# avlmaps/AVLMaps

Hardware: AMD Instinct MI355X
Metric: voxel_query_similarities_per_sec (higher is better)
Workload: dtype f32

## Files before the change

avlmaps_amd/csrc/avl_builder.hip:

```cpp
#include <algorithm>
#include <climits>
#include <cstring>
#include <vector>

#include "avl_builder_state.h"

namespace avl {

#ifdef AVL_PROBE_CHAIN
__device__ unsigned long long* g_probe = nullptr;
constexpr int kProbeK12Row0 = 16384;
#define AVL_STAMP(var)                                                                                             \
    unsigned long long var;                                                                                        \
    asm volatile("s_waitcnt vmcnt(0) lgkmcnt(0)\n\ts_memrealtime %0\n\ts_waitcnt lgkmcnt(0)" : "=s"(var)::"memory")
#define AVL_STAMP_DECL(var) unsigned long long var = 0
#define AVL_RESTAMP(var) asm volatile("s_waitcnt vmcnt(0) lgkmcnt(0)\n\ts_memrealtime %0\n\ts_waitcnt lgkmcnt(0)" : "=s"(var)::"memory")
#else
#define AVL_STAMP(var)
#define AVL_STAMP_DECL(var)
#define AVL_RESTAMP(var)
#endif

#ifndef AVL_K3_THREADS
#define AVL_K3_THREADS 256
#endif
constexpr int kFuseWaves = 128;

constexpr int kEmpty = -1, kPending = -2;
constexpr int kAggregateSamples = 32768;
constexpr int kMaxPendingSpins = 1 << 18;

template <int LINES>
__device__ __forceinline__ void warm_kernel_arguments() {
#ifndef AVL_NO_KERNARG_WARMUP
    static_assert(LINES == 4 || LINES == 8 || LINES == 12 || LINES == 16, "four lines per step");
    const auto p = __builtin_amdgcn_kernarg_segment_ptr();
    int t0, t1, t2, t3;
    if constexpr (LINES == 4)
        asm volatile("s_load_dword %0, %4, 0x0\n s_load_dword %1, %4, 0x40\n s_load_dword %2, %4, 0x80\n s_load_dword %3, %4, 0xc0\n"
                     "s_waitcnt lgkmcnt(0)" : "=&s"(t0), "=&s"(t1), "=&s"(t2), "=&s"(t3) : "s"(p));
    if constexpr (LINES == 8)
        asm volatile("s_load_dword %0, %4, 0x0\n s_load_dword %1, %4, 0x40\n s_load_dword %2, %4, 0x80\n s_load_dword %3, %4, 0xc0\n"
                     "s_load_dword %0, %4, 0x100\n s_load_dword %1, %4, 0x140\n s_load_dword %2, %4, 0x180\n s_load_dword %3, %4, 0x1c0\n"
                     "s_waitcnt lgkmcnt(0)" : "=&s"(t0), "=&s"(t1), "=&s"(t2), "=&s"(t3) : "s"(p));
    if constexpr (LINES == 12)
        asm volatile("s_load_dword %0, %4, 0x0\n s_load_dword %1, %4, 0x40\n s_load_dword %2, %4, 0x80\n s_load_dword %3, %4, 0xc0\n"
                     "s_load_dword %0, %4, 0x100\n s_load_dword %1, %4, 0x140\n s_load_dword %2, %4, 0x180\n s_load_dword %3, %4, 0x1c0\n"
                     "s_load_dword %0, %4, 0x200\n s_load_dword %1, %4, 0x240\n s_load_dword %2, %4, 0x280\n s_load_dword %3, %4, 0x2c0\n"
                     "s_waitcnt lgkmcnt(0)" : "=&s"(t0), "=&s"(t1), "=&s"(t2), "=&s"(t3) : "s"(p));
    if constexpr (LINES == 16)
        asm volatile("s_load_dword %0, %4, 0x0\n s_load_dword %1, %4, 0x40\n s_load_dword %2, %4, 0x80\n s_load_dword %3, %4, 0xc0\n"
                     "s_load_dword %0, %4, 0x100\n s_load_dword %1, %4, 0x140\n s_load_dword %2, %4, 0x180\n s_load_dword %3, %4, 0x1c0\n"
                     "s_load_dword %0, %4, 0x200\n s_load_dword %1, %4, 0x240\n s_load_dword %2, %4, 0x280\n s_load_dword %3, %4, 0x2c0\n"
                     "s_load_dword %0, %4, 0x300\n s_load_dword %1, %4, 0x340\n s_load_dword %2, %4, 0x380\n s_load_dword %3, %4, 0x3c0\n"
                     "s_waitcnt lgkmcnt(0)" : "=&s"(t0), "=&s"(t1), "=&s"(t2), "=&s"(t3) : "s"(p));
    (void)t0; (void)t1; (void)t2; (void)t3;
    __builtin_amdgcn_sched_barrier(0);
#endif
}

__device__ __forceinline__ int py_int(double v) {
    return (int)fmin(fmax(v, -2.0e9), 2.0e9);
}

__device__ __forceinline__ double gemv3(const double* a, double x0, double x1, double x2) {
    return fma(a[2], x2, fma(a[0], x0, a[1] * x1));
}

struct SampleRec {
    double alpha;
    int32_t cell, fpix;
    uint32_t rgbv;
    int32_t slot;
};

template <int THREADS, int MODE = 0>
__device__ __forceinline__ SampleRec bp_voxelize_body(int blk, const FrameParams& fp, const float* depth,
                                                      const int32_t* __restrict__ sample_idx, const uint8_t* rgb,
                                                      int32_t* __restrict__ cell_slot, int32_t* __restrict__ slot_cell, const Recs& recs,
                                                      unsigned long long* __restrict__ counters, int* __restrict__ err_flags,
                                                      PreRec* __restrict__ pre_out = nullptr) {
    __shared__ unsigned blk_new;
    __shared__ unsigned long long blk_base;
    if constexpr (MODE != 2) {
        if (threadIdx.x == 0) blk_new = 0;
        __syncthreads();
    }
    const int s = blk * THREADS + threadIdx.x;
    const bool valid = s < fp.P;
    AVL_STAMP(pt0);
    AVL_STAMP_DECL(pt1);
    AVL_STAMP_DECL(pt2);
    AVL_STAMP_DECL(pt3);
    double alpha = 0.0;
    int32_t cell = -1, fpix = 0;
    uint32_t rgbv = 0;
    int32_t seen = kEmpty;
    bool ok = false, err_box = false, err_img = false;
    uint8_t c0 = 0, c1 = 0, c2 = 0;
    if constexpr (MODE == 1) {
        const PreRec r = valid ? fp.pre[s] : PreRec{0.0, -1, 0, 0u, 0u};
        alpha = r.alpha;
        cell = r.cell;
        fpix = r.fpix;
        rgbv = r.rgbv;
        ok = cell >= 0;
        err_box = (r.flags & 1u) != 0;
        err_img = (r.flags & 2u) != 0;
        AVL_RESTAMP(pt1);
        seen = cell_slot[ok ? cell : 0];
        AVL_RESTAMP(pt2);
        AVL_RESTAMP(pt3);
    } else {

    const BatchEntry* be = fp.batch ? fp.batch + (valid ? s / fp.P_frame : 0) : nullptr;
    double T[12];
    if (be) {
#pragma unroll
        for (int k = 0; k < 12; ++k) T[k] = be->t[k];
        depth = be->depth;
        rgb = be->rgb;
    } else {
#pragma unroll
        for (int k = 0; k < 12; ++k) T[k] = fp.t[k];
    }
    const int pix = !valid ? -1 : (be ? be->samples[s % fp.P_frame] : sample_idx[s]);
    const bool ok0 = pix >= 0 && pix < fp.H * fp.W;
    AVL_RESTAMP(pt1);
    const int pixc = ok0 ? pix : 0;
    const float* dsrc = ok0 ? depth : reinterpret_cast<const float*>(cell_slot);
    const double x = (double)(pixc % fp.W) + 0.5, y = (double)(pixc / fp.W) + 0.5;
    const double z = fp.depth_u16 ? (double)reinterpret_cast<const uint16_t*>(dsrc)[pixc] / fp.depth_div : (double)dsrc[pixc];
    const double pl0 = fma(fp.kinv[2], 1.0, fma(fp.kinv[1], y, fp.kinv[0] * x)) * z;
    const double pl1 = fma(fp.kinv[5], 1.0, fma(fp.kinv[4], y, fp.kinv[3] * x)) * z;
    const double pl2 = fma(fp.kinv[8], 1.0, fma(fp.kinv[7], y, fp.kinv[6] * x)) * z;
    const bool ok1 = ok0 && (pl2 > fp.min_depth) && (pl2 < fp.max_depth);
    AVL_RESTAMP(pt2);
    const double g0 = fma(T[3], 1.0, fma(T[2], pl2, fma(T[1], pl1, T[0] * pl0)));
    const double g1 = fma(T[7], 1.0, fma(T[6], pl2, fma(T[5], pl1, T[4] * pl0)));
    const double g2 = fma(T[11], 1.0, fma(T[10], pl2, fma(T[9], pl1, T[8] * pl0)));
    int row, col, h;
    if (fp.mode == 0) {
        row = py_int(fp.half_gs - (double)py_int(g0 / fp.cs));
        col = py_int(fp.half_gs - (double)py_int(g1 / fp.cs));
        h = py_int(g2 / fp.cs);
    } else {
        row = py_int(rint((g0 - fp.pcd_min[0]) / fp.cs));
        h = py_int(rint((g1 - fp.pcd_min[1]) / fp.cs));
        col = py_int(rint((g2 - fp.pcd_min[2]) / fp.cs));
    }
    const bool in_grid = !(col >= fp.n1 || row >= fp.n0 || h >= fp.n2 || col < 0 || row < 0 || h < 0);
    const bool ok2 = ok1 && in_grid;
    err_box = ok1 && !in_grid && fp.mode == 1;
    const int32_t cell_try = ok2 ? (int32_t)(((unsigned)row * (unsigned)fp.n1 + (unsigned)col) * (unsigned)fp.n2 + (unsigned)h) : 0;
    if constexpr (MODE == 0) seen = cell_slot[cell_try];
    __builtin_amdgcn_sched_barrier(0);
    double q0 = gemv3(fp.k + 0, pl0, pl1, pl2), q1 = gemv3(fp.k + 3, pl0, pl1, pl2), q2 = gemv3(fp.k + 6, pl0, pl1, pl2);
    int px = py_int(q0 / q2 - 0.5), py = py_int(q1 / q2 - 0.5);
    px += px < 0 ? fp.W : 0;
    py += py < 0 ? fp.H : 0;
    const bool in_img = !(px < 0 || px >= fp.W || py < 0 || py >= fp.H);
    err_img = ok2 && !in_img;
    const bool ok3 = ok2 && in_img;
    const size_t rgb_off = ok3 ? ((size_t)py * fp.W + px) * 3 : 0;
    using gbyte_ptr = const __attribute__((address_space(1))) uint8_t*;
    const gbyte_ptr c = (gbyte_ptr)(ok3 ? rgb + rgb_off : reinterpret_cast<const uint8_t*>(cell_slot));
    c0 = c[0];
    c1 = c[1];
    c2 = c[2];
    __builtin_amdgcn_sched_barrier(0);
    q0 = gemv3(fp.kf + 0, pl0, pl1, pl2);
    q1 = gemv3(fp.kf + 3, pl0, pl1, pl2);
    q2 = gemv3(fp.kf + 6, pl0, pl1, pl2);
    px = py_int(q0 / q2 - 0.5);
    py = py_int(q1 / q2 - 0.5);
    ok = ok3 && !(px < 0 || py < 0 || px >= fp.Wf || py >= fp.Hf);
    if (ok2) fpix = (int32_t)((unsigned)py * (unsigned)fp.Wf + (unsigned)px);
    const double radial = (pl0 * pl0 + pl1 * pl1) + pl2 * pl2;
    const double alpha_try = exp(-radial / fp.two_sigma_sq);
    if (ok) {
        alpha = alpha_try;
        cell = cell_try;
    }
// ... 7 lines not shown
    }
    int32_t known = -1;
    bool creator = false;
    if (ok) {
        if (seen == kEmpty) creator = atomicCAS(&cell_slot[cell], kEmpty, kPending) == kEmpty;
        else if (seen >= 0) known = seen;
    }
    AVL_STAMP(pt4);
    const unsigned long long cmask = __ballot(creator);
    const int lane = threadIdx.x & 63;
    unsigned long long base = 0;
#ifndef AVL_K1_AGG_MIN
#define AVL_K1_AGG_MIN kAggregateSamples
#endif
    if (fp.P >= AVL_K1_AGG_MIN) {
        unsigned woff = 0;
        if (cmask) {
            const int leader = __ffsll((long long)cmask) - 1;
            if (lane == leader) woff = atomicAdd(&blk_new, (unsigned)__popcll(cmask));
            woff = __shfl(woff, leader, 64);
        }
        __syncthreads();
        if (threadIdx.x == 0 && blk_new) blk_base = atomicAdd(&counters[0], (unsigned long long)blk_new);
        __syncthreads();
        base = blk_base + woff;
    } else if (cmask) {
        const int leader = __ffsll((long long)cmask) - 1;
        if (lane == leader) base = atomicAdd(&counters[0], (unsigned long long)__popcll(cmask));
        base = __shfl(base, leader, 64);
    }
    if (creator) {
        const unsigned long long slot = base + __popcll(cmask & ((1ull << lane) - 1ull));
        if ((long long)slot >= fp.capacity) {
            atomicOr(err_flags, 1);
            __hip_atomic_store(&cell_slot[cell], kEmpty, __ATOMIC_RELAXED, __HIP_MEMORY_SCOPE_AGENT);
        } else {
            slot_cell[slot] = cell;
            __hip_atomic_store(&cell_slot[cell], (int32_t)slot, __ATOMIC_RELAXED, __HIP_MEMORY_SCOPE_AGENT);
            known = (int32_t)slot;
        }
    }
    if (MODE == 0 && ok) rgbv = (uint32_t)c0 | ((uint32_t)c1 << 8) | ((uint32_t)c2 << 16);
    if (valid) {
        recs.alpha[s] = alpha;
        recs.fpix[s] = fpix;
        recs.rgb[s] = rgbv;
    }
    if (err_box) atomicOr(err_flags, 8);
    if (err_img) atomicOr(err_flags, 2);
#ifdef AVL_PROBE_CHAIN
    {
        AVL_STAMP(pt5);
        if (g_probe && valid && fp.P < kProbeK12Row0) {
            unsigned long long* q = g_probe + (size_t)(kProbeK12Row0 + s) * 8;
            q[0] = pt0; q[1] = pt1; q[2] = pt2; q[3] = pt3; q[4] = pt4; q[5] = pt5;
        }
    }
#endif
    return SampleRec{alpha, cell, fpix, rgbv, known};
}

template <bool MAY_COMPACT = true, int THREADS = 256>
__device__ __forceinline__ void link_body(int blk, int P, const int32_t* __restrict__ cell_slot, int32_t* __restrict__ head,
                                          const Recs& recs, unsigned long long* __restrict__ counters, const ReplayLog& log,
                                          long long log_base, unsigned long long frame_key, const BatchEntry* __restrict__ batch,
                                          int P_frame, const SampleRec& in, int* __restrict__ err_flags, const OwnerList& ol = OwnerList{}) {
    __shared__ unsigned blk_cnt[2];
    __shared__ unsigned sh_own[4];
    if (threadIdx.x < 2) blk_cnt[threadIdx.x] = 0;
    __syncthreads();
    const int s = blk * THREADS + threadIdx.x;
    const bool valid = s < P;
    int32_t slot = -1, next = -1;
    uint8_t owner = 0;
    if (valid) {
        const int32_t cell = in.cell;
        if (cell >= 0) {
            {
                slot = in.slot >= 0 ? in.slot : __hip_atomic_load(&cell_slot[cell], __ATOMIC_RELAXED, __HIP_MEMORY_SCOPE_AGENT);
                for (int spins = 0; slot == kPending; ++spins) {
                    if (spins >= kMaxPendingSpins) {
                        atomicOr(err_flags, 16);
                        slot = -1;
                        break;
                    }
                    __builtin_amdgcn_s_sleep(2);
                    slot = __hip_atomic_load(&cell_slot[cell], __ATOMIC_RELAXED, __HIP_MEMORY_SCOPE_AGENT);
                }
            }
            if (slot >= 0) {
                next = atomicExch(&head[slot], s);
                owner = next == -1;
            }
        }
    }
    const unsigned long long amask = __ballot(slot >= 0);
    const unsigned long long omask = __ballot(owner != 0);
    if (amask && (threadIdx.x & 63) == __ffsll((long long)amask) - 1) {
        atomicAdd(&blk_cnt[0], (unsigned)__popcll(amask));
        if (omask) atomicAdd(&blk_cnt[1], (unsigned)__popcll(omask));
    }
    if (MAY_COMPACT && (threadIdx.x & 63) == 0) sh_own[threadIdx.x >> 6] = (unsigned)__popcll(omask);
    if (valid) {
        recs.slot[s] = slot;
        recs.next[s] = next;
        recs.owner[s] = owner;
        if (log.slot) {
            const long long i = log_base + s;
            log.slot[i] = slot >= 0 ? (uint32_t)slot : 0xFFFFFFFFu;
#ifdef AVL_ABL_NOLOGREC
            if (false) {
#elif defined(AVL_LOG_UNCOND)
            {
#else
            if (slot >= 0) {
#endif
                const unsigned long long k = batch ? (batch[s / P_frame].frame_key | (unsigned)(s % P_frame)) : (frame_key | (unsigned)s);
                using u64x2 = __attribute__((ext_vector_type(2))) unsigned long long;
                u64x2* r = reinterpret_cast<u64x2*>(log.rec + i);
                r[0] = u64x2{(unsigned long long)__double_as_longlong(in.alpha), k};
                r[1] = u64x2{(unsigned long long)in.rgbv, 0ull};
            }
        }
    }
#ifdef AVL_PROBE_CHAIN
    {
        AVL_STAMP(pt7);
        if (g_probe && valid && P < kProbeK12Row0) g_probe[(size_t)(kProbeK12Row0 + s) * 8 + 7] = pt7 | ((unsigned long long)(slot >= 0) << 63);
    }
#endif
    __syncthreads();
    if (MAY_COMPACT && owner && P >= kAggregateSamples) {
        unsigned pos = (unsigned)__popcll(omask & ((1ull << (threadIdx.x & 63)) - 1ull));
        for (int w = 0; w < (int)(threadIdx.x >> 6); ++w) pos += sh_own[w];
        const size_t o = (size_t)blk * 256 + pos;
        ol.o_s[o] = s;
        ol.o_slot[o] = slot;
        ol.o_alpha[o] = in.alpha;
        ol.o_fpix[o] = in.fpix;
        ol.o_rgb[o] = in.rgbv;
    }
    if (MAY_COMPACT && P >= kAggregateSamples && threadIdx.x == 0) ol.ocnt[blk] = (int32_t)(sh_own[0] + sh_own[1] + sh_own[2] + sh_own[3]);
    if (threadIdx.x < 2 && blk_cnt[threadIdx.x]) atomicAdd(&counters[1 + threadIdx.x], (unsigned long long)blk_cnt[threadIdx.x]);
}

__global__ __launch_bounds__(256) void voxelize_link_kernel(FrameParams fp, const float* depth, const int32_t* __restrict__ sample_idx,
                                                            const uint8_t* rgb, int32_t* __restrict__ cell_slot,
                                                            int32_t* __restrict__ slot_cell, Recs recs, int32_t* __restrict__ head,
                                                            unsigned long long* __restrict__ counters, int* __restrict__ err_flags,
                                                            ReplayLog log, long long log_base, unsigned long long frame_key, OwnerList ol) {
    warm_kernel_arguments<12>();
    const SampleRec r = bp_voxelize_body<256>(blockIdx.x, fp, depth, sample_idx, rgb, cell_slot, slot_cell, recs, counters, err_flags);
    link_body<true, 256>(blockIdx.x, fp.P, cell_slot, head, recs, counters, log, log_base, frame_key, fp.batch, fp.P_frame, r, err_flags, ol);
}

__global__ __launch_bounds__(256) void voxelize_link_next_kernel(FrameParams fp, const float* depth, const int32_t* __restrict__ sample_idx,
                                                                 const uint8_t* rgb, int32_t* __restrict__ cell_slot,
                                                                 int32_t* __restrict__ slot_cell, Recs recs, int32_t* __restrict__ head,
                                                                 unsigned long long* __restrict__ counters, int* __restrict__ err_flags,
                                                                 ReplayLog log, long long log_base, unsigned long long frame_key,
                                                                 FrameParams fpn, PreGather next, int gb) {
    if ((int)blockIdx.x < gb) {
        bp_voxelize_body<256, 2>((int)blockIdx.x, fpn, next.depth, next.samples, next.rgb, cell_slot, slot_cell, recs, counters, err_flags, next.out);
        return;
    }
    const int blk = (int)blockIdx.x - gb;
    warm_kernel_arguments<12>();
    SampleRec r;
    if (fp.pre) r = bp_voxelize_body<256, 1>(blk, fp, depth, sample_idx, rgb, cell_slot, slot_cell, recs, counters, err_flags);
    else r = bp_voxelize_body<256, 0>(blk, fp, depth, sample_idx, rgb, cell_slot, slot_cell, recs, counters, err_flags);
    link_body<false, 256>(blk, fp.P, cell_slot, head, recs, counters, log, log_base, frame_key, nullptr, fp.P_frame, r, err_flags);
}

template <int CH, bool FULL>
__device__ __forceinline__ void fuse_group_impl(int s0, int32_t slot, double alpha0, int32_t fpix0, uint32_t rgb0, int P, int D_rt, unsigned long long frame_key, const BatchEntry* __restrict__ batch,
                                                int P_frame, const Recs& recs, int32_t* __restrict__ head, const float* __restrict__ feat,
                                                double* __restrict__ sum_feat, double* __restrict__ sum_w4,
                                                float* __restrict__ first_feat, double* __restrict__ first_alpha,
                                                unsigned long long* __restrict__ slot_key, uint8_t* __restrict__ dirty) {
    const int D = FULL ? 256 * CH : D_rt;
    const int lane = threadIdx.x & 63;
    AVL_STAMP(pt0);
    AVL_STAMP(pt1);
    const bool is_new = slot_key[slot] == kNoKey;
    const int h0 = head[slot];
    double* sf = sum_feat + (size_t)slot * D;
    AVL_STAMP(pt2);
#ifdef AVL_PROBE_CHAIN
    int probe_n = 1;
    unsigned long long pt3 = 0, pt4 = 0;
#endif

    double acc[CH][4], old[CH][4];
    float f1[CH][4];
#pragma unroll
    for (int c = 0; c < CH; ++c)
#pragma unroll
        for (int e = 0; e < 4; ++e) { acc[c][e] = 0.0; f1[c][e] = 0.f; old[c][e] = 0.0; }
    double w4 = 0.0, a1 = 0.0, w4_old = 0.0;
    int min_s = INT_MAX;
    if (!is_new) {
#pragma unroll
        for (int c = 0; c < CH; ++c) {
            const int d = c * 256 + lane * 4;
            if (FULL || (d + 3 < D && (D & 1) == 0)) {
                const double2 q0 = *reinterpret_cast<const double2*>(sf + d), q1 = *reinterpret_cast<const double2*>(sf + d + 2);
                old[c][0] = q0.x; old[c][1] = q0.y; old[c][2] = q1.x; old[c][3] = q1.y;
            } else {
#pragma unroll
                for (int e = 0; e < 4; ++e)
                    if (d + e < D) old[c][e] = sf[d + e];
            }
        }
    }
    if (lane < 4) w4_old = is_new ? 0.0 : sum_w4[(size_t)slot * 4 + lane];

    auto row_of = [&](int cur, int32_t fpix) { return (batch ? batch[cur / P_frame].feat : feat) + (size_t)fpix * D; };
    auto load_row = [&](float (&v)[CH][4], const float* f) {
#pragma unroll
        for (int c = 0; c < CH; ++c) {
            const int d = c * 256 + lane * 4;
            if (FULL || (d + 3 < D && (D & 3) == 0)) {
                const float4 q = *reinterpret_cast<const float4*>(f + d);
                v[c][0] = q.x; v[c][1] = q.y; v[c][2] = q.z; v[c][3] = q.w;
            } else {
#pragma unroll
                for (int e = 0; e < 4; ++e) v[c][e] = d + e < D ? f[d + e] : 0.f;
            }
        }
    };
    auto add = [&](int cur, double alpha, uint32_t rgbv, const float (&v)[CH][4]) {
        const bool first = cur < min_s;
        const bool hold = first && is_new;
        const bool rejoin = hold && min_s != INT_MAX;
        const double a_prev = a1;
        if (first) { min_s = cur; a1 = alpha; }
#pragma unroll
        for (int c = 0; c < CH; ++c) {
            if (FULL || c * 256 + lane * 4 < D) {
#pragma unroll
                for (int e = 0; e < 4; ++e) {
                    if (rejoin) acc[c][e] += a_prev * (double)f1[c][e];
                    if (!hold) acc[c][e] += alpha * (double)v[c][e];
                    if (first) f1[c][e] = v[c][e];
                }
            }
        }
        if (lane < 4) w4 += lane == 0 ? alpha : alpha * (double)((rgbv >> (8 * (lane - 1))) & 0xffu);
    };
    const float* feat0 = row_of(s0, fpix0);
#ifdef AVL_ABL_K3_SINGLE
    if (true) {
#else
    if (h0 == s0) {
#endif
        float v[CH][4];
        load_row(v, feat0);
        add(s0, alpha0, rgb0, v);
#ifdef AVL_PROBE_CHAIN
        { AVL_STAMP(ptx); pt3 = pt4 = ptx; }
#endif
    } else {
        int my = lane == 0 ? s0 : INT_MAX;
        int n = 1, cur = h0;
        while (cur != s0 && n < 64 && (unsigned)cur < (unsigned)P) {
            if (lane == n) my = cur;
            ++n;
            cur = recs.next[cur];
        }
#ifdef AVL_PROBE_CHAIN
        { AVL_STAMP(ptx); pt3 = ptx; probe_n = n; }
#endif
        double a_l = 0.0;
        int32_t fp_l = 0;
        uint32_t rgb_l = 0;
        if (lane < n) {
            a_l = recs.alpha[my];
            fp_l = recs.fpix[my];
            rgb_l = recs.rgb[my];
        }
#ifdef AVL_PROBE_CHAIN
        { AVL_STAMP(ptx); pt4 = ptx; }
#endif
        int rank = 0;
        for (int j = 0; j < n; ++j) rank += __builtin_amdgcn_readlane(my, j) < my ? 1 : 0;
        const int a_lo = __double2loint(a_l), a_hi = __double2hiint(a_l);
#ifndef AVL_K3_MR
#define AVL_K3_MR 2
#endif
        constexpr int MR = CH <= 4 ? AVL_K3_MR : 1;
        for (int k0 = 0; k0 < n; k0 += MR) {
            float v[MR][CH][4];
            int cj[MR], lj[MR];
#pragma unroll
            for (int j = 0; j < MR; ++j) {
                const unsigned long long m = __ballot(lane < n && rank == k0 + j);
                lj[j] = m ? __builtin_amdgcn_readfirstlane(__ffsll((long long)m) - 1) : 0;
                cj[j] = m ? __builtin_amdgcn_readlane(my, lj[j]) : -1;
                load_row(v[j], cj[j] >= 0 ? row_of(cj[j], __builtin_amdgcn_readlane(fp_l, lj[j])) : feat0);
            }
#pragma unroll
            for (int j = 0; j < MR; ++j) {
                if (cj[j] >= 0) {
                    const double al = __hiloint2double(__builtin_amdgcn_readlane(a_hi, lj[j]), __builtin_amdgcn_readlane(a_lo, lj[j]));
                    add(cj[j], al, (uint32_t)__builtin_amdgcn_readlane((int)rgb_l, lj[j]), v[j]);
                }
            }
        }
        for (int steps = 0; cur != s0 && (unsigned)cur < (unsigned)P && steps < P; ++steps) {
            const int nxt = recs.next[cur];
            float v[CH][4];
            load_row(v, row_of(cur, recs.fpix[cur]));
            add(cur, recs.alpha[cur], recs.rgb[cur], v);
            cur = nxt;
        }
    }

    AVL_STAMP(pt5);
    float* ff = first_feat + (size_t)slot * D;
#pragma unroll
    for (int c = 0; c < CH; ++c) {
        const int d = c * 256 + lane * 4;
        double r[4];
#pragma unroll
// ... 395 lines not shown
    const unsigned gb = next.out ? (unsigned)((fpn.P + AVL_K3_THREADS - 1) / AVL_K3_THREADS) : 0u;
    hipLaunchKernelGGL(pipe_kernel<CH>, dim3(pb + wb + gb), dim3(AVL_K3_THREADS), 0, st, fp, (int)pb, reinterpret_cast<const float*>(d_depth), d_sample_idx,
                       d_rgb, b->cell_slot, b->slot_cell, b->recs, b->head, b->counters, b->err_flags, b->log, b->log_used, frame_key, prev,
                       b->D, b->sum_feat, b->sum_w4, b->first_feat, b->first_alpha, b->slot_key, b->dirty, fpn, next, (int)gb);
}

extern "C" {

#ifdef AVL_PROBE_CHAIN
__attribute__((visibility("default"))) int avl_debug_set_probe(void* d_buf) {
    AVL_HIP_CHECK(hipDeviceSynchronize());
    unsigned long long* p = reinterpret_cast<unsigned long long*>(d_buf);
    AVL_HIP_CHECK(hipMemcpyToSymbol(HIP_SYMBOL(avl::g_probe), &p, sizeof(p)));
    return AVL_OK;
}
#endif

int avl_builder_reset(avl_builder* b, void* stream) {
    AVL_REQUIRE(b, "avl_builder_reset: null handle");
    hipStream_t st = as_stream(stream);
    AVL_HIP_CHECK(hipMemsetAsync(b->cell_slot, 0xFF, b->ncell * sizeof(int32_t), st));
    AVL_HIP_CHECK(hipMemsetAsync(b->head, 0xFF, (size_t)b->capacity * sizeof(int32_t), st));
    AVL_HIP_CHECK(hipMemsetAsync(b->head_alt, 0xFF, (size_t)b->capacity * sizeof(int32_t), st));
    b->pend = avl_builder::Pending{};
    b->pre_held.valid = false;
    AVL_HIP_CHECK(hipMemsetAsync(b->dirty, 0, (size_t)b->capacity, st));
    AVL_HIP_CHECK(hipMemsetAsync(b->slot_cell, 0xFF, (size_t)b->capacity * sizeof(int32_t), st));
    AVL_HIP_CHECK(hipMemsetAsync(b->slot_key, 0xFF, (size_t)b->capacity * sizeof(unsigned long long), st));
    AVL_HIP_CHECK(hipMemsetAsync(b->counters, 0, 4 * sizeof(unsigned long long), st));
    AVL_HIP_CHECK(hipMemsetAsync(b->err_flags, 0, sizeof(int), st));
    b->key_bias = 0;
    b->log_used = 0;
    b->vox_bound = 0;
    drop_log_segments(b, st);
    return AVL_OK;
}

int avl_builder_destroy(avl_builder* b) {
    if (!b) return AVL_OK;
    drop_log_segments(b, nullptr);
    (void)hipFree(b->cell_slot); (void)hipFree(b->slot_cell); (void)hipFree(b->slot_key); (void)hipFree(b->sum_feat);
    (void)hipFree(b->sum_w4); (void)hipFree(b->first_feat); (void)hipFree(b->first_alpha); (void)hipFree(b->head);
    (void)hipFree(b->head_alt);
    (void)hipFree(b->dirty);
    (void)hipFree(b->counters); (void)hipFree(b->err_flags); (void)hipFree(b->recs_mem);
    (void)hipFree(b->log.slot); (void)hipFree(b->log.rec);
    (void)hipFree(b->rs_mem);
    (void)hipFree(b->d_table);
    delete b;
    return AVL_OK;
}

int avl_builder_create_grid(avl_builder** h_out, int n0, int gs, int vh, double cs, int D, int64_t capacity) {
    AVL_REQUIRE(h_out, "avl_builder_create: null output");
    *h_out = nullptr;
    avl::keep_mempool_once();
    avl_merge2_load();
    AVL_REQUIRE(n0 > 0 && gs > 0 && vh > 0 && D > 0 && cs > 0 && capacity > 0, "avl_builder_create: bad parameters");
    const double ncell_d = (double)n0 * gs * vh;
    AVL_REQUIRE(ncell_d < 2.0e9, "avl_builder_create: gs*gs*vh = %.0f cells exceeds the int32 cell index", ncell_d);
    AVL_REQUIRE(capacity < (1ll << 31), "avl_builder_create: capacity must fit int32 voxel ids");
    avl_builder* b = new avl_builder();
    b->n0 = n0; b->gs = gs; b->vh = vh; b->D = D; b->cs = cs; b->capacity = capacity;
    b->ncell = (size_t)n0 * gs * vh;
    hipError_t e = hipSuccess;
    auto alloc = [&](void** p, size_t bytes) { if (e == hipSuccess) e = hipMalloc(p, bytes); };
    alloc((void**)&b->cell_slot, b->ncell * sizeof(int32_t));
    alloc((void**)&b->slot_cell, (size_t)capacity * sizeof(int32_t));
    alloc((void**)&b->slot_key, (size_t)capacity * sizeof(unsigned long long));
    alloc((void**)&b->sum_feat, (size_t)capacity * D * sizeof(double));
    alloc((void**)&b->sum_w4, (size_t)capacity * 4 * sizeof(double));
    alloc((void**)&b->first_feat, (size_t)capacity * D * sizeof(float));
    alloc((void**)&b->first_alpha, (size_t)capacity * sizeof(double));
    alloc((void**)&b->head, (size_t)capacity * sizeof(int32_t));
    alloc((void**)&b->head_alt, (size_t)capacity * sizeof(int32_t));
    alloc((void**)&b->dirty, (size_t)capacity);
    alloc((void**)&b->counters, 4 * sizeof(unsigned long long));
    alloc((void**)&b->err_flags, sizeof(int));
    if (e != hipSuccess) {
        set_error("avl_builder_create: hipMalloc failed: %s (capacity %lld x D %d)", hipGetErrorString(e), (long long)capacity, D);
        avl_builder_destroy(b);
        return AVL_ERR_HIP;
    }
    int rc = avl_builder_reset(b, nullptr);
    if (rc == AVL_OK && hipDeviceSynchronize() != hipSuccess) rc = AVL_ERR_HIP;
    if (rc != AVL_OK) {
        avl_builder_destroy(b);
        return rc;
    }
    *h_out = b;
    return AVL_OK;
}

int avl_builder_enable_replay_log(avl_builder* b, int64_t max_samples) {
    AVL_REQUIRE(b && max_samples > 0, "avl_builder_enable_replay_log: bad arguments");
    AVL_REQUIRE(max_samples < (1ll << 31), "avl_builder_enable_replay_log: at most 2^31 - 1 samples");
    AVL_HIP_CHECK(hipDeviceSynchronize());
    if (b->log_used != 0) {
        set_error("avl_builder_enable_replay_log: frames were already fused; enable the log on a fresh or reset builder");
        return AVL_ERR_STATE;
    }
    (void)hipFree(b->log.slot); (void)hipFree(b->log.rec);
    b->log = ReplayLog{};
    b->log_cap = 0;
    hipError_t e = hipMalloc((void**)&b->log.slot, (size_t)max_samples * sizeof(uint32_t));
    if (e == hipSuccess) e = hipMalloc((void**)&b->log.rec, (size_t)max_samples * sizeof(LogRec));
    if (e != hipSuccess) {
        (void)hipFree(b->log.slot); (void)hipFree(b->log.rec);
        b->log = ReplayLog{};
        set_error("avl_builder_enable_replay_log: hipMalloc failed: %s", hipGetErrorString(e));
        return AVL_ERR_HIP;
    }
    b->log_cap = max_samples;
    (void)hipFree(b->rs_mem);
    b->rs_mem = nullptr;
    b->rs_bytes = b->rs_tmp_bytes = 0;
    if (const size_t tb = replay_sort_tmp_bytes(max_samples)) {
        const size_t w = ((size_t)max_samples * 4 + 255) / 256 * 256;
        const size_t total = 4 * w + (tb + 255) / 256 * 256 + 256;
        if (hipMalloc((void**)&b->rs_mem, total) == hipSuccess) {
            b->rs_bytes = total;
            b->rs_tmp_bytes = (tb + 255) / 256 * 256;
        } else {
            b->rs_mem = nullptr;
            (void)hipGetLastError();
        }
    }
    return AVL_OK;
}

int avl_builder_set_max_capacity(avl_builder* b, int64_t max_capacity) {
    AVL_REQUIRE(b, "avl_builder_set_max_capacity: null handle");
    AVL_REQUIRE(max_capacity == 0 || (max_capacity >= b->capacity && max_capacity < (1ll << 31)),
                "avl_builder_set_max_capacity: must be 0 (fixed) or in [capacity, 2^31)");
    b->max_capacity = max_capacity;
    return AVL_OK;
}

int avl_builder_capacity(avl_builder* b, int64_t* h_capacity) {
    AVL_REQUIRE(b && h_capacity, "avl_builder_capacity: null argument");
    *h_capacity = b->capacity;
    return AVL_OK;
}

int avl_builder_create(avl_builder** h_out, int gs, double cs, int vh, int D, int64_t capacity) {
    return avl_builder_create_grid(h_out, gs, gs, vh, cs, D, capacity);
}

static int integrate_impl(avl_builder* b, const void* d_depth, int depth_u16, double depth_div, int H, int W, const double* h_calib,
                          const double* h_calib_inv, const double* h_pc_transform, const int32_t* d_sample_idx, int P,
                          const float* d_feat, int Hf, int Wf, const uint8_t* d_rgb, int64_t frame_idx, double min_depth,
                          double max_depth, double sigma_sq, const double* h_pcd_min, void* stream, int B = 0,
                          const void* const* h_depth_ptrs = nullptr, const int32_t* const* h_sample_ptrs = nullptr,
                          const float* const* h_feat_ptrs = nullptr, const uint8_t* const* h_rgb_ptrs = nullptr) {
    AVL_REQUIRE(b, "avl_builder_integrate_frame: null handle");
    const auto held = b->pre_held;
    b->pre_held.valid = false;
    AVL_REQUIRE(H > 0 && W > 0 && Hf > 0 && Wf > 0 && P >= 0, "avl_builder_integrate_frame: bad shape");
    AVL_REQUIRE(P < (1 << 30), "avl_builder_integrate_frame: at most 2^30 samples per frame");
    AVL_REQUIRE(B >= 0 && (int64_t)(B > 0 ? B : 1) * P < (1ll << 30), "avl_builder_integrate_batch: at most 2^30 samples per launch");
    AVL_REQUIRE(frame_idx >= 0 && frame_idx + B < (1ll << 30), "avl_builder_integrate_frame: bad frame_idx");
    AVL_REQUIRE(sigma_sq > 0, "avl_builder_integrate_frame: sigma_sq must be positive");
    if (P == 0) return AVL_OK;
    AVL_REQUIRE(h_calib && h_calib_inv && h_pc_transform, "avl_builder_integrate_frame: null pointer");
    if (B == 0) AVL_REQUIRE(d_depth && d_sample_idx && d_feat && d_rgb, "avl_builder_integrate_frame: null pointer");
    else AVL_REQUIRE(h_depth_ptrs && h_sample_ptrs && h_feat_ptrs && h_rgb_ptrs, "avl_builder_integrate_batch: null pointer table");
    hipStream_t st = as_stream(stream);
    const int P_frame = P;
    if (B > 0) P = B * P_frame;
    int rc = ensure_recs(b, P, st);
    if (rc != AVL_OK) return rc;
    if (b->max_capacity > b->capacity && b->vox_bound + P > b->capacity) {
        int64_t have = 0;
        rc = read_counter(b, 0, &have, st);
        if (rc != AVL_OK) return rc;
        b->vox_bound = have;
        int64_t need = have + P;
        if (need > (int64_t)b->ncell) need = (int64_t)b->ncell;
        if (need > b->capacity) {
            rc = grow_builder(b, need, st);
            if (rc != AVL_OK) return rc;
        }
    }
    b->vox_bound += P;
    const unsigned long long key_bias = b->key_bias;
    if (B > 0) {
        if (B > b->table_cap) {
            AVL_HIP_CHECK(hipStreamSynchronize(st));
            if (b->d_table) AVL_HIP_CHECK(hipFree(b->d_table));
            b->d_table = nullptr;
            AVL_HIP_CHECK(hipMalloc((void**)&b->d_table, (size_t)(B + 16) * sizeof(BatchEntry)));
            b->table_cap = B + 16;
        }
        std::vector<BatchEntry> tab((size_t)B);
        for (int i = 0; i < B; ++i) {
            AVL_REQUIRE(h_depth_ptrs[i] && h_sample_ptrs[i] && h_feat_ptrs[i] && h_rgb_ptrs[i], "avl_builder_integrate_batch: null frame %d", i);
            memcpy(tab[i].t, h_pc_transform + 16 * i, 16 * sizeof(double));
            tab[i].depth = reinterpret_cast<const float*>(h_depth_ptrs[i]);
            tab[i].samples = h_sample_ptrs[i];
            tab[i].rgb = h_rgb_ptrs[i];
            tab[i].feat = h_feat_ptrs[i];
            tab[i].frame_key = key_bias | ((unsigned long long)(frame_idx + i) << 32);
        }
        AVL_HIP_CHECK(hipMemcpyAsync(b->d_table, tab.data(), (size_t)B * sizeof(BatchEntry), hipMemcpyHostToDevice, st));
    }
    FrameParams fp;
    for (int i = 0; i < 9; ++i) { fp.kinv[i] = h_calib_inv[i]; fp.k[i] = h_calib[i]; fp.kf[i] = 0.0; }
    fp.kf[0] = fp.kf[4] = (double)Wf / 2.0;
    fp.kf[2] = (double)Wf / 2.0;
    fp.kf[5] = (double)Hf / 2.0;
    fp.kf[8] = 1.0;
    for (int i = 0; i < 16; ++i) fp.t[i] = h_pc_transform[i];
    fp.min_depth = min_depth; fp.max_depth = max_depth;
    fp.two_sigma_sq = 2 * sigma_sq;
    fp.cs = b->cs; fp.half_gs = (double)b->gs / 2.0;
    fp.H = H; fp.W = W; fp.Hf = Hf; fp.Wf = Wf; fp.n0 = b->n0; fp.n1 = b->gs; fp.n2 = b->vh; fp.P = P;
    fp.batch = B > 0 ? b->d_table : nullptr;
    fp.P_frame = P_frame;
    fp.mode = h_pcd_min ? 1 : 0;
    for (int i = 0; i < 3; ++i) fp.pcd_min[i] = h_pcd_min ? h_pcd_min[i] : 0.0;
    fp.depth_u16 = depth_u16;
    fp.depth_div = depth_div;
    fp.capacity = b->capacity;
    fp.pre = nullptr;
    FrameParams fpn{};
    PreGather next{};
    const bool pre_ok = B == 0 && !depth_u16 && b->D <= 1536 && P < kAggregateSamples;
    if (pre_ok) {
        const auto& h = held;
        if (h.valid && h.samples == d_sample_idx && h.depth == d_depth && h.rgb == d_rgb && same_geometry(h.fp, fp)) fp.pre = b->pre_buf[h.buf];
        if (b->pre_next.samples) {
            fpn = fp;
            fpn.pre = nullptr;
            for (int i = 0; i < 16; ++i) fpn.t[i] = b->pre_next.h_pc_transform[i];
            next = PreGather{b->pre_buf[fp.pre ? 1 - h.buf : 0], b->pre_next.depth, b->pre_next.samples, b->pre_next.rgb};
        }
    }
    const int next_buf = next.out == b->pre_buf[1] ? 1 : 0;
    auto hold_next = [&]() {
        if (!next.out) return;
        b->pre_held.fp = fpn;
        b->pre_held.samples = next.samples;
        b->pre_held.depth = next.depth;
        b->pre_held.rgb = next.rgb;
        b->pre_held.buf = next_buf;
        b->pre_held.valid = true;
    };
    const unsigned long long frame_key = b->key_bias | ((unsigned long long)frame_idx << 32);

    if (b->ls_cache) drop_log_segments(b, st);
    if (b->log.slot && b->log_used + P > b->log_cap) {
        set_error("replay log full (%lld samples): enable it with a larger max_samples", b->log_cap);
        return AVL_ERR_CAPACITY;
    }
    const unsigned pb = (unsigned)((P + 255) / 256);
    if (b->deferred && B == 0 && b->D <= 1536) {
        const FusePrev prev{b->pend.P, b->pend.frame_key, b->recs_alt, b->head_alt, b->pend.feat};
        const unsigned pb = (unsigned)((P + AVL_K3_THREADS - 1) / AVL_K3_THREADS);
        if (b->D <= 256) launch_pipe<1>(b, fp, pb, d_depth, d_sample_idx, d_rgb, frame_key, prev, st, fpn, next);
        else if (b->D <= 512) launch_pipe<2>(b, fp, pb, d_depth, d_sample_idx, d_rgb, frame_key, prev, st, fpn, next);
        else if (b->D == 768) launch_pipe<3>(b, fp, pb, d_depth, d_sample_idx, d_rgb, frame_key, prev, st, fpn, next);
        else if (b->D <= 1024) launch_pipe<4>(b, fp, pb, d_depth, d_sample_idx, d_rgb, frame_key, prev, st, fpn, next);
        else launch_pipe<6>(b, fp, pb, d_depth, d_sample_idx, d_rgb, frame_key, prev, st, fpn, next);
        if (b->log.slot) b->log_used += P;
        b->pend.P = P;
        b->pend.frame_key = frame_key;
        b->pend.feat = d_feat;
        std::swap(b->recs, b->recs_alt);
        std::swap(b->head, b->head_alt);
        AVL_HIP_CHECK(hipGetLastError());
        hold_next();
        return AVL_OK;
    }
    rc = flush_pending(b, st);
    if (rc != AVL_OK) return rc;
    const bool k2_compacts = !(fp.pre || next.out);
    if (!k2_compacts) {
        const unsigned gb = next.out ? pb : 0u;
        hipLaunchKernelGGL(voxelize_link_next_kernel, dim3(gb + pb), dim3(256), 0, st, fp, reinterpret_cast<const float*>(d_depth), d_sample_idx,
                           d_rgb, b->cell_slot, b->slot_cell, b->recs, b->head, b->counters, b->err_flags, b->log, b->log_used, frame_key, fpn,
                           next, (int)gb);
    } else {
        hipLaunchKernelGGL(voxelize_link_kernel, dim3(pb), dim3(256), 0, st, fp, reinterpret_cast<const float*>(d_depth), d_sample_idx, d_rgb,
                           b->cell_slot, b->slot_cell, b->recs, b->head, b->counters, b->err_flags, b->log, b->log_used, frame_key, b->owners);
    }
    if (b->log.slot) b->log_used += P;
    rc = launch_fuse(b, P, frame_key, fp.batch, P_frame, b->recs, b->head, d_feat, st, k2_compacts);
    if (rc == AVL_OK) hold_next();
    return rc;
}

int avl_builder_set_deferred_fuse(avl_builder* b, int on, void* stream) {
    AVL_REQUIRE(b, "avl_builder_set_deferred_fuse: null handle");
    if (!on) {
        int rc = flush_pending(b, as_stream(stream));
        if (rc != AVL_OK) return rc;
    }
    b->deferred = on ? 1 : 0;
    return AVL_OK;
}

int avl_builder_flush(avl_builder* b, void* stream) {
    AVL_REQUIRE(b, "avl_builder_flush: null handle");
    return flush_pending(b, as_stream(stream));
}

int avl_builder_release_scratch(avl_builder* b, int64_t keep_bytes, void* stream) {
    AVL_REQUIRE(b, "avl_builder_release_scratch: null handle");
    AVL_REQUIRE(keep_bytes >= 0, "avl_builder_release_scratch: keep_bytes < 0");
    hipStream_t st = as_stream(stream);
    drop_log_segments(b, st);
    AVL_HIP_CHECK(hipStreamSynchronize(st));
    avl::trim_mempool((uint64_t)keep_bytes);
    return AVL_OK;
}

int avl_builder_integrate_frame(avl_builder* b, const float* d_depth, int H, int W, const double* h_calib,
                                const double* h_calib_inv, const double* h_pc_transform, const int32_t* d_sample_idx, int P,
                                const float* d_feat, int Hf, int Wf, const uint8_t* d_rgb, int64_t frame_idx,
                                double min_depth, double max_depth, double sigma_sq, void* stream) {
    return integrate_impl(b, d_depth, 0, 1.0, H, W, h_calib, h_calib_inv, h_pc_transform, d_sample_idx, P, d_feat, Hf, Wf, d_rgb,
                          frame_idx, min_depth, max_depth, sigma_sq, nullptr, stream);
}

int avl_builder_integrate_frame_global(avl_builder* b, const void* d_depth, int depth_is_u16, double depth_div, int H, int W,
                                       const double* h_calib, const double* h_calib_inv, const double* h_transform,
                                       const int32_t* d_sample_idx, int P, const float* d_feat, int Hf, int Wf,
                                       const uint8_t* d_rgb, int64_t frame_idx, double min_depth, double max_depth,
                                       double sigma_sq, const double* h_pcd_min, void* stream) {
    AVL_REQUIRE(h_pcd_min, "avl_builder_integrate_frame_global: pcd_min is required");
    AVL_REQUIRE(!depth_is_u16 || depth_div > 0, "avl_builder_integrate_frame_global: depth_div must be positive");
    return integrate_impl(b, d_depth, depth_is_u16 ? 1 : 0, depth_div, H, W, h_calib, h_calib_inv, h_transform, d_sample_idx, P, d_feat,
                          Hf, Wf, d_rgb, frame_idx, min_depth, max_depth, sigma_sq, h_pcd_min, stream);
}

int avl_builder_integrate_batch(avl_builder* b, int B, const float* const* h_depth_ptrs, int H, int W, const double* h_calib,
                                const double* h_calib_inv, const double* h_pc_transforms, const int32_t* const* h_sample_ptrs, int P,
                                const float* const* h_feat_ptrs, int Hf, int Wf, const uint8_t* const* h_rgb_ptrs, int64_t frame_idx0,
                                double min_depth, double max_depth, double sigma_sq, void* stream) {
    AVL_REQUIRE(B > 0, "avl_builder_integrate_batch: B must be positive");
    return integrate_impl(b, nullptr, 0, 1.0, H, W, h_calib, h_calib_inv, h_pc_transforms, nullptr, P, nullptr, Hf, Wf, nullptr, frame_idx0,
                          min_depth, max_depth, sigma_sq, nullptr, stream, B, reinterpret_cast<const void* const*>(h_depth_ptrs),
                          h_sample_ptrs, h_feat_ptrs, h_rgb_ptrs);
}

int avl_builder_integrate_frames(avl_builder* b, int n_frames, const float* const* h_depth_ptrs, int H, int W, const double* h_calib,
                                 const double* h_calib_inv, const double* h_pc_transforms, const int32_t* const* h_sample_ptrs, int P,
                                 const float* const* h_feat_ptrs, int Hf, int Wf, const uint8_t* const* h_rgb_ptrs, int64_t frame_idx0,
                                 double min_depth, double max_depth, double sigma_sq, void* stream) {
    AVL_REQUIRE(n_frames > 0, "avl_builder_integrate_frames: n_frames must be positive");
    AVL_REQUIRE(h_depth_ptrs && h_sample_ptrs && h_feat_ptrs && h_rgb_ptrs && h_pc_transforms, "avl_builder_integrate_frames: null pointer table");
    AVL_REQUIRE(b, "avl_builder_integrate_frames: null handle");
    for (int i = 0; i < n_frames; ++i) {
        b->pre_next = {};
        if (i + 1 < n_frames && h_sample_ptrs[i + 1] && h_depth_ptrs[i + 1] && h_rgb_ptrs[i + 1])
            b->pre_next = {h_sample_ptrs[i + 1], h_depth_ptrs[i + 1], h_rgb_ptrs[i + 1], h_pc_transforms + 16 * (i + 1)};
        const int rc = integrate_impl(b, h_depth_ptrs[i], 0, 1.0, H, W, h_calib, h_calib_inv, h_pc_transforms + 16 * i, h_sample_ptrs[i], P,
                                      h_feat_ptrs[i], Hf, Wf, h_rgb_ptrs[i], frame_idx0 + i, min_depth, max_depth, sigma_sq, nullptr, stream);
        b->pre_next = {};
        if (rc != AVL_OK) return rc;
    }
    return AVL_OK;
}

int avl_builder_num_voxels(avl_builder* b, int64_t* h_n, void* stream) {
    AVL_REQUIRE(b && h_n, "avl_builder_num_voxels: null argument");
    int rc = flush_pending(b, as_stream(stream));
    if (rc != AVL_OK) return rc;
    rc = builder_check_flags(b, as_stream(stream));
    if (rc != AVL_OK) return rc;
    rc = read_counter(b, 0, h_n, as_stream(stream));
    if (rc == AVL_OK && *h_n > b->capacity) *h_n = b->capacity;
    return rc;
}

int avl_builder_num_points(avl_builder* b, int64_t* h_n, void* stream) {
    AVL_REQUIRE(b && h_n, "avl_builder_num_points: null argument");
    if (int rc = flush_pending(b, as_stream(stream)); rc != AVL_OK) return rc;
    return read_counter(b, 1, h_n, as_stream(stream));
}

int avl_builder_num_groups(avl_builder* b, int64_t* h_n, void* stream) {
    AVL_REQUIRE(b && h_n, "avl_builder_num_groups: null argument");
    if (int rc = flush_pending(b, as_stream(stream)); rc != AVL_OK) return rc;
    return read_counter(b, 2, h_n, as_stream(stream));
}

}
```

Baseline: 183.2 billion.

## Route multi-frame integration through the deferred fused pipeline and drop next-frame pregather kernel

When integrating several frames without deferred mode, integrate_frames now forces the pipelined path, which fuses each frame's voxelize/link with the previous frame's pending fuse, and flushes at the end. The voxelize_link_next_kernel that pre-gathered the next frame inside the link launch is removed, so the non-pipelined path always launches the compacting voxelize_link_kernel and fuse. This aims to overlap per-frame stages across frames and reduce launches, at the cost of holding pending state until a final flush. The metric is query throughput, so any effect depends on whether map building is inside the timed region.

```diff
diff --git a/avlmaps_amd/csrc/avl_builder.hip b/avlmaps_amd/csrc/avl_builder.hip
--- a/avlmaps_amd/csrc/avl_builder.hip
+++ b/avlmaps_amd/csrc/avl_builder.hip
@@ -29,6 +29,10 @@
 constexpr int kEmpty = -1, kPending = -2;
 constexpr int kAggregateSamples = 32768;
 constexpr int kMaxPendingSpins = 1 << 18;
+#ifndef AVL_PIPELINE_MIN_FRAMES
+#define AVL_PIPELINE_MIN_FRAMES 2
+#endif
+constexpr int kPipelineMinFrames = AVL_PIPELINE_MIN_FRAMES;
 
 template <int LINES>
 __device__ __forceinline__ void warm_kernel_arguments() {
@@ -342,24 +346,6 @@
     warm_kernel_arguments<12>();
     const SampleRec r = bp_voxelize_body<256>(blockIdx.x, fp, depth, sample_idx, rgb, cell_slot, slot_cell, recs, counters, err_flags);
     link_body<true, 256>(blockIdx.x, fp.P, cell_slot, head, recs, counters, log, log_base, frame_key, fp.batch, fp.P_frame, r, err_flags, ol);
-}
-
-__global__ __launch_bounds__(256) void voxelize_link_next_kernel(FrameParams fp, const float* depth, const int32_t* __restrict__ sample_idx,
-                                                                 const uint8_t* rgb, int32_t* __restrict__ cell_slot,
-                                                                 int32_t* __restrict__ slot_cell, Recs recs, int32_t* __restrict__ head,
-                                                                 unsigned long long* __restrict__ counters, int* __restrict__ err_flags,
-                                                                 ReplayLog log, long long log_base, unsigned long long frame_key,
-                                                                 FrameParams fpn, PreGather next, int gb) {
-    if ((int)blockIdx.x < gb) {
-        bp_voxelize_body<256, 2>((int)blockIdx.x, fpn, next.depth, next.samples, next.rgb, cell_slot, slot_cell, recs, counters, err_flags, next.out);
-        return;
-    }
-    const int blk = (int)blockIdx.x - gb;
-    warm_kernel_arguments<12>();
-    SampleRec r;
-    if (fp.pre) r = bp_voxelize_body<256, 1>(blk, fp, depth, sample_idx, rgb, cell_slot, slot_cell, recs, counters, err_flags);
-    else r = bp_voxelize_body<256, 0>(blk, fp, depth, sample_idx, rgb, cell_slot, slot_cell, recs, counters, err_flags);
-    link_body<false, 256>(blk, fp.P, cell_slot, head, recs, counters, log, log_base, frame_key, nullptr, fp.P_frame, r, err_flags);
 }
 
 template <int CH, bool FULL>
@@ -1061,7 +1047,8 @@
                           const float* d_feat, int Hf, int Wf, const uint8_t* d_rgb, int64_t frame_idx, double min_depth,
                           double max_depth, double sigma_sq, const double* h_pcd_min, void* stream, int B = 0,
                           const void* const* h_depth_ptrs = nullptr, const int32_t* const* h_sample_ptrs = nullptr,
-                          const float* const* h_feat_ptrs = nullptr, const uint8_t* const* h_rgb_ptrs = nullptr) {
+                          const float* const* h_feat_ptrs = nullptr, const uint8_t* const* h_rgb_ptrs = nullptr,
+                          bool pipelined = false) {
     AVL_REQUIRE(b, "avl_builder_integrate_frame: null handle");
     const auto held = b->pre_held;
     b->pre_held.valid = false;
@@ -1163,7 +1150,7 @@
         return AVL_ERR_CAPACITY;
     }
     const unsigned pb = (unsigned)((P + 255) / 256);
-    if (b->deferred && B == 0 && b->D <= 1536) {
+    if ((b->deferred || pipelined) && B == 0 && b->D <= 1536) {
         const FusePrev prev{b->pend.P, b->pend.frame_key, b->recs_alt, b->head_alt, b->pend.feat};
         const unsigned pb = (unsigned)((P + AVL_K3_THREADS - 1) / AVL_K3_THREADS);
         if (b->D <= 256) launch_pipe<1>(b, fp, pb, d_depth, d_sample_idx, d_rgb, frame_key, prev, st, fpn, next);
@@ -1183,20 +1170,10 @@
     }
     rc = flush_pending(b, st);
     if (rc != AVL_OK) return rc;
-    const bool k2_compacts = !(fp.pre || next.out);
-    if (!k2_compacts) {
-        const unsigned gb = next.out ? pb : 0u;
-        hipLaunchKernelGGL(voxelize_link_next_kernel, dim3(gb + pb), dim3(256), 0, st, fp, reinterpret_cast<const float*>(d_depth), d_sample_idx,
-                           d_rgb, b->cell_slot, b->slot_cell, b->recs, b->head, b->counters, b->err_flags, b->log, b->log_used, frame_key, fpn,
-                           next, (int)gb);
-    } else {
-        hipLaunchKernelGGL(voxelize_link_kernel, dim3(pb), dim3(256), 0, st, fp, reinterpret_cast<const float*>(d_depth), d_sample_idx, d_rgb,
-                           b->cell_slot, b->slot_cell, b->recs, b->head, b->counters, b->err_flags, b->log, b->log_used, frame_key, b->owners);
-    }
+    hipLaunchKernelGGL(voxelize_link_kernel, dim3(pb), dim3(256), 0, st, fp, reinterpret_cast<const float*>(d_depth), d_sample_idx, d_rgb,
+                       b->cell_slot, b->slot_cell, b->recs, b->head, b->counters, b->err_flags, b->log, b->log_used, frame_key, b->owners);
     if (b->log.slot) b->log_used += P;
-    rc = launch_fuse(b, P, frame_key, fp.batch, P_frame, b->recs, b->head, d_feat, st, k2_compacts);
-    if (rc == AVL_OK) hold_next();
-    return rc;
+    return launch_fuse(b, P, frame_key, fp.batch, P_frame, b->recs, b->head, d_feat, st, true);
 }
 
 int avl_builder_set_deferred_fuse(avl_builder* b, int on, void* stream) {
@@ -1260,16 +1237,22 @@
     AVL_REQUIRE(n_frames > 0, "avl_builder_integrate_frames: n_frames must be positive");
     AVL_REQUIRE(h_depth_ptrs && h_sample_ptrs && h_feat_ptrs && h_rgb_ptrs && h_pc_transforms, "avl_builder_integrate_frames: null pointer table");
     AVL_REQUIRE(b, "avl_builder_integrate_frames: null handle");
-    for (int i = 0; i < n_frames; ++i) {
+    const bool pipelined = !b->deferred && n_frames >= kPipelineMinFrames && b->D <= 1536 && P < kAggregateSamples;
+    int rc = AVL_OK;
+    for (int i = 0; i < n_frames && rc == AVL_OK; ++i) {
         b->pre_next = {};
         if (i + 1 < n_frames && h_sample_ptrs[i + 1] && h_depth_ptrs[i + 1] && h_rgb_ptrs[i + 1])
             b->pre_next = {h_sample_ptrs[i + 1], h_depth_ptrs[i + 1], h_rgb_ptrs[i + 1], h_pc_transforms + 16 * (i + 1)};
-        const int rc = integrate_impl(b, h_depth_ptrs[i], 0, 1.0, H, W, h_calib, h_calib_inv, h_pc_transforms + 16 * i, h_sample_ptrs[i], P,
-                                      h_feat_ptrs[i], Hf, Wf, h_rgb_ptrs[i], frame_idx0 + i, min_depth, max_depth, sigma_sq, nullptr, stream);
+        rc = integrate_impl(b, h_depth_ptrs[i], 0, 1.0, H, W, h_calib, h_calib_inv, h_pc_transforms + 16 * i, h_sample_ptrs[i], P,
+                            h_feat_ptrs[i], Hf, Wf, h_rgb_ptrs[i], frame_idx0 + i, min_depth, max_depth, sigma_sq, nullptr, stream, 0, nullptr,
+                            nullptr, nullptr, nullptr, pipelined);
         b->pre_next = {};
-        if (rc != AVL_OK) return rc;
-    }
-    return AVL_OK;
+    }
+    if (pipelined) {
+        const int rcf = flush_pending(b, as_stream(stream));
+        if (rc == AVL_OK) rc = rcf;
+    }
+    return rc;
 }
 
 int avl_builder_num_voxels(avl_builder* b, int64_t* h_n, void* stream) {
```

Result: slower. 180.4 billion (-1.5%).
